# LucaHermes/ddrl

Hardware: AMD Instinct MI355X
Metric: env-steps/sec at 4096 envs × 4 leg agents; PPO update ms/minibatch (higher is better)
Workload: dtype fp32

## Files before the change

### ddrl_amd/csrc/ppo_ffn_impl.h

```cpp
#pragma once
#include <atomic>
#include "common.h"
#include "kernels.h"
#include "ffn.h"
#include "ppo_loss.h"

#ifndef DDRL_FFN_AT
#define DDRL_FFN_AT 0
#endif

#ifndef DDRL_FFN_KSP
#define DDRL_FFN_KSP 0
#endif
#if DDRL_FFN_KSP == 1
#define DDRL_FFN_LAUNCH launch_update_ffn_k1
#elif DDRL_FFN_AT == 2
#define DDRL_FFN_LAUNCH launch_update_ffn_peer
#elif DDRL_FFN_AT
#define DDRL_FFN_LAUNCH launch_update_ffn_atomic
#else
#define DDRL_FFN_LAUNCH launch_update_ffn
#endif
#if DDRL_FFN_AT || defined(DDRL_XCHG_ATOMIC)
#define DDRL_XCHG_IS_ATOMIC 1
#else
#define DDRL_XCHG_IS_ATOMIC 0
#endif
#define DDRL_XCHG_LXSYS (DDRL_FFN_AT == 2)
#define DDRL_LX_ON (!DDRL_XCHG_IS_ATOMIC || DDRL_XCHG_LXSYS)

namespace {

typedef float float2v __attribute__((ext_vector_type(2)));

template <int NW, int ROWS>
struct Geo {
  static constexpr int NT = 64 * NW;
  static constexpr int RT = ROWS / (16 * NW);
  static constexpr int NS1 = 16 / NW;
  static constexpr int NS2 = (12 + NW - 1) / NW;
};
__host__ __device__ constexpr int waves_for(int A, int ksp) { return ksp == 2 ? 4 : (A == 8 ? 4 : 8); }
__host__ __device__ constexpr int ncup_slots(int OB, bool pol) { return pol && OB == 4 ? 2 * OB : 0; }
__host__ __device__ constexpr int gx_pairs(int OB, int NW) {
  return ((64 * OB + OB + 128 + ncup_slots(OB, true) + 64 * NW - 1) / (64 * NW) + 2) / 2 + 2 * (16 / NW + (12 + NW - 1) / NW);
}
#define GX_MAX_PAIRS 20

struct UpdateBatch {
  UpdateArgs a[DDRL_MAXP];
  UpdateHyper h;
  int nrows;
  float inv_n;
  unsigned long long* xchg;
  unsigned long long* gx;
  int* err;
  int* xcc;
  unsigned epoch;
  unsigned lds_bytes;
  int own_kq;
  unsigned lx_base;
};

#ifdef DDRL_BOUNDS
__device__ unsigned g_bounds[DDRL_NBOUNDS];
__device__ __forceinline__ bool bchk(bool ok, int k) {
  if (!ok) atomicAdd(&g_bounds[k], 1u);
  return ok;
}
}
#if !DDRL_FFN_AT
#if DDRL_FFN_KSP == 2
extern "C" int ddrl_diag_bounds_k1(unsigned* host, int reset);
#endif
#if DDRL_FFN_KSP == 1
extern "C" int ddrl_diag_bounds_k1(unsigned* host, int reset) {
#else
extern "C" int ddrl_diag_bounds(unsigned* host, int reset) {
#endif
  if (hipMemcpyFromSymbol(host, HIP_SYMBOL(g_bounds), sizeof(g_bounds)) != hipSuccess) return -1;
  if (reset) {
    unsigned z[DDRL_NBOUNDS] = {0};
    if (hipMemcpyToSymbol(HIP_SYMBOL(g_bounds), z, sizeof(z)) != hipSuccess) return -1;
  }
#if DDRL_FFN_KSP == 2
  unsigned k1[DDRL_NBOUNDS];
  if (ddrl_diag_bounds_k1(k1, reset) != 0) return -1;
  for (int i = 0; i < DDRL_NBOUNDS; ++i) host[i] += k1[i];
#endif
  return 0;
}
#endif
namespace {
#define BCHK(cond, k) bchk((cond), (k))
#else
#define BCHK(cond, k) true
#endif
__device__ __forceinline__ unsigned xchg_tag(unsigned epoch, int step) {
  return (epoch << 20) | (((unsigned)step + 1u) & 0xfffffu);
}

struct BranchOff { int w1, b1, w2, b2, wo, bo, cup; };
__device__ __forceinline__ BranchOff branch_off(const FfnOffsets& o, bool pol) {
  BranchOff b;
  b.cup = o.n;
  b.w1 = pol ? o.w1 : o.vw1; b.b1 = pol ? o.b1 : o.vb1;
  b.w2 = pol ? o.w2 : o.vw2; b.b2 = pol ? o.b2 : o.vb2;
  b.wo = pol ? o.wo : o.vo;  b.bo = pol ? o.bo : o.vbo;
  return b;
}

template <int OB, bool PAD>
__device__ void stage_branch(const float* __restrict__ th, int d, const BranchOff& bo, float* lds,
                             NetLds& W, int ncup) {
  W.w1 = lds; W.w2 = W.w1 + lds_img(48, PAD); W.b1 = W.w2 + lds_img(64, PAD); W.b2 = W.b1 + 64;
  W.wo = W.b2 + 64; W.bo = W.wo + 64 * OB; W.cup = W.bo + OB;
  for (int i = threadIdx.x; i < ncup; i += blockDim.x) W.cup[i] = th[bo.cup + i];
  for (int i = threadIdx.x; i < 48 * 64; i += blockDim.x) {
    const int f = i >> 6;
    W.w1[sidx<PAD>(f, i & 63)] = f < d ? th[bo.w1 + i] : 0.f;
  }
  for (int i = threadIdx.x; i < 64 * 64; i += blockDim.x) W.w2[sidx<PAD>(i >> 6, i & 63)] = th[bo.w2 + i];
  for (int i = threadIdx.x; i < 64; i += blockDim.x) { W.b1[i] = th[bo.b1 + i]; W.b2[i] = th[bo.b2 + i]; }
  for (int i = threadIdx.x; i < 64 * OB; i += blockDim.x) W.wo[i] = th[bo.wo + i];
  for (int i = threadIdx.x; i < OB; i += blockDim.x) W.bo[i] = th[bo.bo + i];
}
template <int OB, int NT, bool PAD>
__device__ __forceinline__ void stage_branch_batched(const float* __restrict__ th, int d, const BranchOff& bo,
                                                     float* lds, NetLds& W, int ncup) {
  static_assert((48 * 64) % NT == 0 && (64 * 64) % NT == 0, "staging split");
  constexpr int N1 = 48 * 64 / NT, N2 = 64 * 64 / NT, NS = (64 * OB + OB + 128 + NT - 1) / NT;
  W.w1 = lds; W.w2 = W.w1 + lds_img(48, PAD); W.b1 = W.w2 + lds_img(64, PAD); W.b2 = W.b1 + 64;
  W.wo = W.b2 + 64; W.bo = W.wo + 64 * OB; W.cup = W.bo + OB;
  const int t = threadIdx.x;
  float a1[N1], a2[N2], as[NS];
#pragma unroll
  for (int k = 0; k < N1; ++k) {
    const int i = t + NT * k;
    a1[k] = (i >> 6) < d ? th[bo.w1 + i] : 0.f;
  }
#pragma unroll
  for (int k = 0; k < N2; ++k) a2[k] = th[bo.w2 + t + NT * k];
#pragma unroll
  for (int k = 0; k < NS; ++k) {
    int e = t + NT * k;
    float x = 0.f;
    if (e < 64 * OB) x = th[bo.wo + e];
    else if ((e -= 64 * OB) < OB) x = th[bo.bo + e];
    else if ((e -= OB) < 64) x = th[bo.b1 + e];
    else if ((e -= 64) < 64) x = th[bo.b2 + e];
    as[k] = x;
  }
  float ac = t < ncup ? th[bo.cup + t] : 0.f;
#pragma unroll
  for (int k = 0; k < N1; ++k) {
    const int i = t + NT * k;
    W.w1[sidx<PAD>(i >> 6, i & 63)] = a1[k];
  }
#pragma unroll
  for (int k = 0; k < N2; ++k) {
    const int i = t + NT * k;
    W.w2[sidx<PAD>(i >> 6, i & 63)] = a2[k];
  }
#pragma unroll
  for (int k = 0; k < NS; ++k) {
    int e = t + NT * k;
    if (e < 64 * OB) W.wo[e] = as[k];
    else if ((e -= 64 * OB) < OB) W.bo[e] = as[k];
    else if ((e -= OB) < 64) W.b1[e] = as[k];
    else if ((e -= 64) < 64) W.b2[e] = as[k];
  }
  if (t < ncup) W.cup[t] = ac;
}
__host__ __device__ constexpr int branch_lds_floats(bool pad) { return lds_img(48, pad) + lds_img(64, pad) + 128 + 64 * 16 + 16; }
__host__ __device__ constexpr bool update_pad(int A, int ksp) { return kLdsPad && !(A == 8 && ksp == 1); }

template <int OB>
__device__ __forceinline__ void small_param(int e, const BranchOff& bo, const NetLds& W, int& pidx, float*& lp) {
  if (e < 64 * OB) { pidx = bo.wo + e; lp = W.wo + e; return; }
  e -= 64 * OB;
  if (e < OB) { pidx = bo.bo + e; lp = W.bo + e; return; }
  e -= OB;
  if (e < 64) { pidx = bo.b1 + e; lp = W.b1 + e; return; }
  e -= 64;
  if (e < 64) { pidx = bo.b2 + e; lp = W.b2 + e; return; }
  e -= 64;
  pidx = bo.cup + e; lp = W.cup + e;
}


template <int A, int RT>
struct RowData {
  float x[RT][12];
  float act[RT][A];
  float ol[RT][2 * A];
  float s0[RT], s1[RT];
  int cid[RT];
};

template <int NW, int ROWS>
__device__ __forceinline__ void issue_rows(const float* rec, int stride, int cpr, int cpr_l, float inv_cpr_l,
                                           const int* idxb, float* stg, int R, unsigned lds_bytes) {
  const int lane = threadIdx.x & 63, w = __builtin_amdgcn_readfirstlane(threadIdx.x >> 6);
  if (w == NW - 1) return;
  constexpr int MI = (ROWS * 20 + 64 * (NW - 1) - 1) / (64 * (NW - 1));
  const int nchunk = ROWS * cpr_l;
  int idx[MI], kk[MI];
#pragma unroll
  for (int it = 0; it < MI; ++it) {
    const int g = 64 * w + 64 * (NW - 1) * it + lane;
    int row = (int)(((float)g + 0.5f) * inv_cpr_l);
    kk[it] = min(g - row * cpr_l, cpr - 1);
    idx[it] = 0;
    if (g < nchunk) {
      if (!BCHK(row >= 0 && row < ROWS && kk[it] >= 0, 0)) row = 0;
      idx[it] = idxb[row];
    }
  }
#pragma unroll
  for (int it = 0; it < MI; ++it) {
    const int base = 64 * w + 64 * (NW - 1) * it;
    if (base >= nchunk) break;
    const unsigned dst = __builtin_amdgcn_readfirstlane(lds_addr(stg + 4 * base));
    if (base + lane < nchunk) {
      int i = idx[it];
      if (!BCHK(i >= 0 && i < R, 1)) i = 0;
      if (BCHK(dst + 16u * (unsigned)lane + 16u <= lds_bytes, 3))
        glds16(rec + (size_t)i * stride + 4 * kk[it], dst);
    }
  }
  (void)R; (void)lds_bytes;
}

__host__ __device__ constexpr int stg_chunks(int stride, int A) { return A == 8 ? stride / 4 : (stride / 4) | 1; }

template <int A, int KS1, bool POL, int RT>
__device__ __forceinline__ void load_row(const float* stg, int stg_stride, const RecLayout& L, const int* row_l,
                                         int d, RowData<A, RT>& r, unsigned xlast_bits = 0xffffffffu) {
  const int q = (threadIdx.x & 63) >> 4;
#ifdef DDRL_BOUNDS
  {
    int hi = KS1 < 12 ? L.obs + 4 * KS1 - 1 : L.obs + d - 1;
    if (POL) hi = max(max(hi, L.act + A - 1), max(L.logit + 2 * A - 1, max(L.logp, max(L.adv, L.cid))));
    else hi = max(hi, max(L.vf, L.vt));
    for (int t = 0; t < RT; ++t) BCHK(row_l[t] >= 0 && row_l[t] < DDRL_MB && hi < L.stride, 4);
  }
#endif
#pragma unroll
  for (int t = 0; t < RT; ++t) {
    const float* rp = stg + row_l[t] * stg_stride;
#pragma unroll
    for (int s = 0; s < 12; ++s)
      r.x[t][s] = (s < KS1 && (KS1 < 12 || 4 * s + q < d)) ? rp[L.obs + 4 * s + q] : 0.f;
    if (KS1 < 12) r.x[t][KS1 - 1] = __uint_as_float(__float_as_uint(r.x[t][KS1 - 1]) & xlast_bits);
    if (POL) {
#pragma unroll
      for (int j = 0; j < A; ++j) r.act[t][j] = rp[L.act + j];
#pragma unroll
      for (int j = 0; j < 2 * A; ++j) r.ol[t][j] = rp[L.logit + j];
      r.s0[t] = rp[L.logp];
      r.s1[t] = rp[L.adv];
      r.cid[t] = L.cid >= 0 ? min(max((int)rp[L.cid], 0), 3) : 0;
    } else {
      r.cid[t] = 0;
#pragma unroll
      for (int j = 0; j < A; ++j) r.act[t][j] = 0.f;
#pragma unroll
      for (int j = 0; j < 2 * A; ++j) r.ol[t][j] = 0.f;
      r.s0[t] = rp[L.vf];
      r.s1[t] = rp[L.vt];
    }
  }
}

template <bool POL, int NSTAT, int NW, int KSP>
__device__ __forceinline__ void write_stats(float* so, const float* red, float inv_n) {
  float sv[NSTAT];
#pragma unroll
  for (int k = 0; k < NSTAT; ++k) {
    if constexpr (KSP == 2) {
      sv[k] = red[96 + k];
    } else {
      sv[k] = 0.f;
      for (int i = 0; i < NW; ++i) sv[k] += red[i * 8 + k];
    }
  }
  if constexpr (POL) {
    gst(so + 1, sv[0] * inv_n); gst(so + 3, sv[1] * inv_n); gst(so + 4, sv[2] * inv_n);
  } else {
    gst(so + 2, sv[0] * inv_n);
    const float vy = sv[2] * inv_n - (sv[1] * inv_n) * (sv[1] * inv_n);
    const float vd = sv[4] * inv_n - (sv[3] * inv_n) * (sv[3] * inv_n);
    gst(so + 5, vy > 0.f ? fmaxf(-1.f, 1.f - vd / vy) : 0.f);
  }
}

__device__ __forceinline__ int row_index(const UpdateArgs& U, int step, int row_l, bool ok) {
  if (!ok) return 0;
  if (!U.shuffle) return row_l;
  const int e = step / U.nb, b = step - e * U.nb;
#ifdef DDRL_BOUNDS
  if (!BCHK(e >= 0 && e < U.n_epochs, 2)) return 0;
  const int slot = gld(U.perm + e * U.nb + b);
  if (!BCHK(slot >= 0 && slot < U.nb && (slot + 1) * DDRL_MB <= max(U.R, DDRL_MB) && row_l < DDRL_MB, 2)) return 0;
  return gld(U.shuffle + slot * DDRL_MB + row_l);
#else
  return gld(U.shuffle + gld(U.perm + e * U.nb + b) * DDRL_MB + row_l);
#endif
}
__device__ __forceinline__ int perm_slot(const UpdateArgs& U, int step) {
  const int e = step / U.nb, b = step - e * U.nb;
  return gld(U.perm + e * U.nb + b);
}

#ifdef DDRL_STAMPS
__device__ unsigned long long g_stamps[32][16];
#define STAMP_INIT unsigned long long st_prev = __builtin_amdgcn_s_memtime(), st_acc[16] = {0};
#ifndef DDRL_STAMP_TID
#define DDRL_STAMP_TID 0
#endif
#define STAMP(k) do { if (tid == DDRL_STAMP_TID) { const unsigned long long t_ = __builtin_amdgcn_s_memtime(); st_acc[k] += t_ - st_prev; st_prev = t_; } } while (0)
#define STAMP_DONE do { if (tid == DDRL_STAMP_TID) for (int k_ = 0; k_ < 16; ++k_) g_stamps[blockIdx.x][k_] = st_acc[k_]; } while (0)
}
#if !DDRL_FFN_AT && DDRL_FFN_KSP != 1
extern "C" int ddrl_diag_stamps(unsigned long long* host) {
  return hipMemcpyFromSymbol(host, HIP_SYMBOL(g_stamps), sizeof(g_stamps)) == hipSuccess ? 0 : -1;
}
#endif
namespace {
#else
#define STAMP_INIT
#define STAMP(k)
#define STAMP_DONE
#endif

constexpr int kGxSt = 0, kGxLd = 16;
#define XCHG_SLOW_TICKS 20000ull
#define XCHG_TIMEOUT_TICKS 300000000ull
__device__ __forceinline__ bool xchg_abandon(unsigned long long t0, int* err) {
  const unsigned long long dt = __builtin_amdgcn_s_memrealtime() - t0;
  if (dt < XCHG_SLOW_TICKS) return false;
  if (__hip_atomic_load(err, __ATOMIC_RELAXED, __HIP_MEMORY_SCOPE_AGENT)) return true;
  if (dt > XCHG_TIMEOUT_TICKS) { atomicExch(err, 1); return true; }
  return false;
}
#if DDRL_XCHG_IS_ATOMIC
#define DDRL_XCHG_SCOPE __HIP_MEMORY_SCOPE_SYSTEM
typedef unsigned long long* gx_box_t;
__device__ __forceinline__ gx_box_t gx_rsrc(unsigned long long* box) { return box; }
__device__ __forceinline__ void gx_put(gx_box_t r, int j, float v0, float v1, unsigned tag, bool) {
  unsigned long long* g = r + 2 * (j * 256 + (int)threadIdx.x);
  __hip_atomic_store(g, ((unsigned long long)tag << 32) | __float_as_uint(v0), __ATOMIC_RELAXED, DDRL_XCHG_SCOPE);
  __hip_atomic_store(g + 1, ((unsigned long long)tag << 32) | __float_as_uint(v1), __ATOMIC_RELAXED,
                     DDRL_XCHG_SCOPE);
}
__device__ __forceinline__ void xchg_store(unsigned long long* g, unsigned long long v, bool) {
  __hip_atomic_store(g, v, __ATOMIC_RELAXED, DDRL_XCHG_SCOPE);
}
__device__ __forceinline__ unsigned long long xchg_load(unsigned long long* g) {
  return __hip_atomic_load(g, __ATOMIC_RELAXED, DDRL_XCHG_SCOPE);
}
template <int NP, typename F>
__device__ __forceinline__ bool gx_get(gx_box_t r, unsigned tag, float* out, int* err, F&& after_first) {
  bool lost = false;
  unsigned long long g[2 * NP];
  unsigned long long* b = r + 2 * (int)threadIdx.x;
  const unsigned long long t0 = __builtin_amdgcn_s_memrealtime();
  bool first = true;
  for (;;) {
#pragma unroll
    for (int j = 0; j < NP; ++j) {
      g[2 * j] = __hip_atomic_load(b + 512 * j, __ATOMIC_RELAXED, DDRL_XCHG_SCOPE);
      g[2 * j + 1] = __hip_atomic_load(b + 512 * j + 1, __ATOMIC_RELAXED, DDRL_XCHG_SCOPE);
    }
    if (first) { after_first(); first = false; }
    bool ok = true;
#pragma unroll
    for (int j = 0; j < 2 * NP; ++j) ok = ok && (unsigned)(g[j] >> 32) == tag;
    if (ok) break;
    if (xchg_abandon(t0, err)) {
#pragma unroll
      for (int j = 0; j < 2 * NP; ++j) g[j] = 0ull;
      lost = true;
      break;
    }
    __builtin_amdgcn_s_sleep(1);
  }
#pragma unroll
  for (int j = 0; j < 2 * NP; ++j) out[j] = __uint_as_float((unsigned)g[j]);
  return lost;
}
#else
typedef __amdgpu_buffer_rsrc_t gx_box_t;
__device__ __forceinline__ gx_box_t gx_rsrc(unsigned long long* box) {
  return __builtin_amdgcn_make_buffer_rsrc(box, 0, GX_MAX_PAIRS * 256 * 16, 0x00020000);
}
__device__ __forceinline__ void gx_put(gx_box_t r, int j, float v0, float v1, unsigned tag, bool coh) {
  const v4u g = {__float_as_uint(v0), tag, __float_as_uint(v1), tag};
  if (coh) __builtin_amdgcn_raw_buffer_store_b128(g, r, (j * 256 + (int)threadIdx.x) * 16, 0, 16);
  else __builtin_amdgcn_raw_buffer_store_b128(g, r, (j * 256 + (int)threadIdx.x) * 16, 0, kGxSt);
}
__device__ __forceinline__ void xchg_store(unsigned long long* g, unsigned long long v, bool coh) {
  const __amdgpu_buffer_rsrc_t r = __builtin_amdgcn_make_buffer_rsrc(g, 0, 8, 0x00020000);
  typedef unsigned v2u_t __attribute__((ext_vector_type(2)));
  const v2u_t x = {(unsigned)v, (unsigned)(v >> 32)};
  if (coh) __builtin_amdgcn_raw_buffer_store_b64(x, r, 0, 0, 16);
  else __builtin_amdgcn_raw_buffer_store_b64(x, r, 0, 0, kGxSt);
}
__device__ __forceinline__ unsigned long long xchg_load(unsigned long long* g) {
  const __amdgpu_buffer_rsrc_t r = __builtin_amdgcn_make_buffer_rsrc(g, 0, 8, 0x00020000);
  typedef unsigned v2u_t __attribute__((ext_vector_type(2)));
  const v2u_t x = __builtin_amdgcn_raw_buffer_load_b64(r, 0, 0, kGxLd);
  return ((unsigned long long)x[1] << 32) | x[0];
}
template <int NP, typename F>
__device__ __forceinline__ bool gx_get(gx_box_t r, unsigned tag, float* out, int* err, F&& after_first) {
  bool lost = false;
  v4u g[NP];
  const unsigned long long t0 = __builtin_amdgcn_s_memrealtime();
  bool first = true;
  for (;;) {
#pragma unroll
    for (int j = 0; j < NP; ++j) g[j] = __builtin_amdgcn_raw_buffer_load_b128(r, (j * 256 + (int)threadIdx.x) * 16, 0, kGxLd);
    if (first) { after_first(); first = false; }
    bool ok = true;
#pragma unroll
    for (int j = 0; j < NP; ++j) ok = ok && g[j][1] == tag && g[j][3] == tag;
    if (ok) break;
    if (xchg_abandon(t0, err)) {
#pragma unroll
      for (int j = 0; j < NP; ++j) g[j] = v4u{0u, 0u, 0u, 0u};
      lost = true;
      break;
    }
    __builtin_amdgcn_s_sleep(1);
  }
#pragma unroll
  for (int j = 0; j < NP; ++j) {
    out[2 * j] = __uint_as_float(g[j][0]);
    out[2 * j + 1] = __uint_as_float(g[j][2]);
  }
  return lost;
}
#endif

__device__ __forceinline__ unsigned lx_bit(int step) { return ((unsigned)(step >> 1) & 1u) ^ 1u; }
__device__ __forceinline__ float lx_t(float v, unsigned bit) { return __uint_as_float((__float_as_uint(v) & ~1u) | bit); }
#if DDRL_LX_ON
#if DDRL_XCHG_LXSYS
typedef __amdgpu_buffer_rsrc_t lx_box_t;
__device__ __forceinline__ lx_box_t lx_rsrc(unsigned long long* box) {
  return __builtin_amdgcn_make_buffer_rsrc(box, 0, GX_MAX_PAIRS * 256 * 16, 0x00020000);
}
constexpr int kLxSt = 17, kLxLd = 17;
#else
typedef gx_box_t lx_box_t;
__device__ __forceinline__ lx_box_t lx_rsrc(unsigned long long* box) { return gx_rsrc(box); }
constexpr int kLxSt = kGxSt, kLxLd = kGxLd;
#endif
__device__ __forceinline__ void gx_put4(lx_box_t r, int j, float a, float b, float c, float d, unsigned bit) {
  const v4u g = {__float_as_uint(lx_t(a, bit)), __float_as_uint(lx_t(b, bit)), __float_as_uint(lx_t(c, bit)),
                 __float_as_uint(lx_t(d, bit))};
  __builtin_amdgcn_raw_buffer_store_b128(g, r, (j * 256 + (int)threadIdx.x) * 16, 0, kLxSt);
}
template <int NQ, typename F>
__device__ __forceinline__ bool gx_get4(lx_box_t r, unsigned bit, float* out, int* err, F&& after_first) {
  bool lost = false;
  v4u g[NQ];
  const unsigned long long t0 = __builtin_amdgcn_s_memrealtime();
  bool first = true;
  for (;;) {
#pragma unroll
    for (int j = 0; j < NQ; ++j) g[j] = __builtin_amdgcn_raw_buffer_load_b128(r, (j * 256 + (int)threadIdx.x) * 16, 0, kLxLd);
    if (first) { after_first(); first = false; }
    unsigned bad = 0;
#pragma unroll
    for (int j = 0; j < NQ; ++j) bad |= (g[j][0] ^ bit) | (g[j][1] ^ bit) | (g[j][2] ^ bit) | (g[j][3] ^ bit);
    if ((bad & 1u) == 0) break;
    if (xchg_abandon(t0, err)) {
#pragma unroll
      for (int j = 0; j < NQ; ++j) g[j] = v4u{0u, 0u, 0u, 0u};
      lost = true;
      break;
    }
    __builtin_amdgcn_s_sleep(1);
  }
#pragma unroll
  for (int j = 0; j < NQ; ++j)
#pragma unroll
    for (int k = 0; k < 4; ++k) out[4 * j + k] = __uint_as_float(g[j][k]);
  return lost;
}
#endif

template <int O>
__device__ __forceinline__ void head_bwd_mfma(const NetLds& W, const float* dout, floatx4 dh[4]) {
  static_assert(O % 4 == 0, "policy head: 2A outputs");
  const int lane = threadIdx.x & 63, c = lane & 15, q = lane >> 4;
  float b[O / 4];
#pragma unroll
  for (int kk = 0; kk < O / 4; ++kk)
    b[kk] = q == 0 ? dout[4 * kk] : q == 1 ? dout[4 * kk + 1] : q == 2 ? dout[4 * kk + 2] : dout[4 * kk + 3];
#pragma unroll
  for (int fb = 0; fb < 4; ++fb) {
    floatx4 acc = splat4(0.f);
#pragma unroll
    for (int kk = 0; kk < O / 4; ++kk) acc = mfma4(W.wo[(16 * fb + c) * O + 4 * kk + q], b[kk], acc);
    dh[fb] = acc;
  }
}

template <int NROWS, int NT_, int LD = NROWS + 8>
__device__ __forceinline__ void dw_tiles_fm_head(const float* A, const float* B, const int* fa, int fo, floatx4* out,
                                                 const float* AH, const float* BH, int fah, floatx4& outh) {
  const int lane = threadIdx.x & 63, c = lane & 15, q = lane >> 4;
#pragma unroll
  for (int i = 0; i < NT_; ++i) out[i] = splat4(0.f);
  outh = splat4(0.f);
  const float* bp = B + (16 * fo + c) * LD + 4 * q;
  const float* bph = BH + c * LD + 4 * q;
  const float* aph = AH + (16 * fah + c) * LD + 4 * q;
  const float* ap[NT_];
#pragma unroll
  for (int i = 0; i < NT_; ++i) ap[i] = A + (16 * fa[i] + c) * LD + 4 * q;
  constexpr int NU = NROWS / 16;
  floatx4 bv[2], av[2][NT_], bhv[2], ahv[2];
  bv[0] = *reinterpret_cast<const floatx4*>(bp);
  bhv[0] = *reinterpret_cast<const floatx4*>(bph);
  ahv[0] = *reinterpret_cast<const floatx4*>(aph);
#pragma unroll
  for (int i = 0; i < NT_; ++i) av[0][i] = *reinterpret_cast<const floatx4*>(ap[i]);
#pragma unroll
  for (int u = 0; u < NU; ++u) {
    if (u + 1 < NU) {
      bv[(u + 1) & 1] = *reinterpret_cast<const floatx4*>(bp + 16 * (u + 1));
      bhv[(u + 1) & 1] = *reinterpret_cast<const floatx4*>(bph + 16 * (u + 1));
      ahv[(u + 1) & 1] = *reinterpret_cast<const floatx4*>(aph + 16 * (u + 1));
#pragma unroll
      for (int i = 0; i < NT_; ++i) av[(u + 1) & 1][i] = *reinterpret_cast<const floatx4*>(ap[i] + 16 * (u + 1));
    }
#pragma unroll
    for (int v = 0; v < 4; ++v) {
#pragma unroll
      for (int i = 0; i < NT_; ++i) out[i] = mfma4(av[u & 1][i][v], bv[u & 1][v], out[i]);
      outh = mfma4(ahv[u & 1][v], bhv[u & 1][v], outh);
    }
    __builtin_amdgcn_sched_barrier(0);
  }
}

template <int A, int KS1, int OB, bool POL, int NW, int KSP, bool CUP, bool LSBX>
__device__ __forceinline__ void update_loop(const UpdateArgs& U, const UpdateBatch& ub, float* lds, int p, int kq) {
  constexpr int ROWS = DDRL_MB / KSP;
  constexpr int NT = Geo<NW, ROWS>::NT, RT = Geo<NW, ROWS>::RT, NS1 = Geo<NW, ROWS>::NS1, NS2 = Geo<NW, ROWS>::NS2;
  constexpr bool PAD = update_pad(A, KSP);
  const int wkq = ub.own_kq < 0 ? 0 : ub.own_kq;
  const UpdateHyper& H = ub.h;
  const int d = U.d;
  const FfnOffsets of = ffn_offsets(d, A);
  const BranchOff bo = branch_off(of, POL);
  const int nf1 = (d + 15) >> 4;
  constexpr int NSB0 = 64 * OB + OB + 128;
  constexpr int NCUP = CUP ? ncup_slots(OB, POL) : 0;
  constexpr int NSB = NSB0 + NCUP;
  constexpr bool cup = NCUP > 0;
  constexpr int nsb = NSB;
  constexpr int NSLOT = (NSB + NT - 1) / NT;
  constexpr int NSTAT = POL ? 3 : 5;
  constexpr int NTS = NS1 + NS2;
  constexpr int NP0 = (NSLOT + 2) / 2;
  constexpr int NP = NP0 + 2 * NTS;
  static_assert(KSP == 1 || (NT == 256 && NP == gx_pairs(OB, NW) && NP <= GX_MAX_PAIRS), "exchange pairs");
  constexpr bool LX = LSBX && KSP == 2 && DDRL_LX_ON;
  constexpr int NQ0 = (NSLOT + 1 + 3) / 4;
  constexpr int NQ = NQ0 + NTS;
  static_assert(!LX || NQ <= GX_MAX_PAIRS, "exchange quads");

  NetLds W;
  constexpr int LD = ROWS + 8;
  float* bufA = lds + branch_lds_floats(PAD);
  float* bufB = bufA + 64 * LD;
  float* Pb = bufB + 64 * LD;
  float* red = Pb + NW * NSB;
  int* idxb = reinterpret_cast<int*>(red + 128);
  constexpr bool HMF = POL && KSP == 2;
  float* bufH = red + 256;
  float* bufD = bufH + 64 * LD;
  float* stg = red + 256 + (HMF ? 80 * LD : 0);
  const int stride = U.lay.stride, cpr = stride >> 2, cpr_l = stg_chunks(stride, A);
  const float inv_cpr_l = 1.f / (float)cpr_l;

  const int tid = threadIdx.x, lane = tid & 63, c = lane & 15, q = lane >> 4,
            w = __builtin_amdgcn_readfirstlane(tid >> 6);
  constexpr bool coh = false;
  int row_l[RT];
  bool row_ok[RT];
#pragma unroll
  for (int t = 0; t < RT; ++t) {
    row_l[t] = 16 * RT * w + 16 * t + c;
    row_ok[t] = ROWS * kq + row_l[t] < ub.nrows;
  }

  const int total_steps = U.n_epochs * U.nb;
  const int last = U.max_steps >= 0 ? min(total_steps, U.step0 + U.max_steps) : total_steps;
  const int gr = ROWS * kq + tid;
  const bool gok = tid < ROWS && gr < ub.nrows;
  if (tid < ROWS) idxb[tid] = U.step0 < last && gok ? row_index(U, U.step0, gr, true) : 0;
  __syncthreads();
  if (U.step0 < last) issue_rows<NW, ROWS>(U.rec, stride, cpr, cpr_l, inv_cpr_l, idxb, stg, U.R, ub.lds_bytes);
  stage_branch_batched<OB, NT, PAD>(U.theta, d, bo, lds, W, NCUP);
  if constexpr (HMF) {
    for (int i = tid; i < NW * NSB; i += NT) Pb[i] = 0.f;
    for (int i = tid; i < 16 * LD; i += NT) bufD[i] = 0.f;
  }

  floatx4 mt[NTS], vt4[NTS];
  bool tv[NTS];
  int tfa[NTS], tfo[NTS];
#pragma unroll
  for (int i = 0; i < NTS; ++i) {
    const int tt = i < NS1 ? w + NW * i : w + NW * (i - NS1);
    tv[i] = i < NS1 ? true : (tt < 4 * nf1);
    tfa[i] = tt >> 2;
    tfo[i] = tt & 3;
#pragma unroll
    for (int r = 0; r < 4; ++r) {
      const int f = 16 * tfa[i] + 4 * q + r, o = 16 * tfo[i] + c;
      const bool ok = tv[i] && (i < NS1 || f < d) && !U.grad_out;
      const int pidx = (i < NS1 ? bo.w2 : bo.w1) + f * 64 + o;
      BCHK(!ok || (pidx >= 0 && pidx < of.n), 5);
      mt[i][r] = ok ? U.m[pidx] : 0.f;
      vt4[i][r] = ok ? U.v[pidx] : 0.f;

    }
  }
  float ms[NSLOT], vs[NSLOT];
  int sp_pidx[NSLOT], sp_lds[NSLOT];
#pragma unroll
  for (int k = 0; k < NSLOT; ++k) {
    const int e = tid + NT * k;
    ms[k] = vs[k] = 0.f;
    sp_pidx[k] = 0;
    sp_lds[k] = (int)(red + 127 - lds);
    if (e < nsb) {
      int pidx; float* lp;
      small_param<OB>(e, bo, W, pidx, lp);
      BCHK(pidx >= 0 && pidx < of.n + NCUP, 5);
      sp_pidx[k] = pidx;
      sp_lds[k] = (int)(lp - lds);
      if (!U.grad_out) {
        ms[k] = U.m[pidx];
        vs[k] = U.v[pidx];
      }
    }
  }
  int ebase[4];
#pragma unroll
  for (int r = 0; r < 4; ++r) ebase[r] = sidx<PAD>(4 * q + r, 16 * (w & 3) + c);
  float b1p = U.beta_pow[0], b2p = U.beta_pow[1];
  const float adv_mean = U.adv_norm[0], adv_den = U.adv_norm[1];
  const float beta = U.kl_coeff;
  const float lo = 1.f - H.clip, hi = 1.f + H.clip;
  __syncthreads();

  RowData<A, RT> cur;
  const unsigned xlast_bits = (KS1 < 12 && 4 * (KS1 - 1) + q >= d) ? 0u : 0xffffffffu;
  wait_vmcnt0();
  __syncthreads();
  if (tid < ROWS) idxb[tid] = U.step0 + 1 < last && gok ? row_index(U, U.step0 + 1, gr, true) : 0;
  int nxt = U.step0 + 2 < last && gok ? row_index(U, U.step0 + 2, gr, true) : 0;
  const size_t gx_branch = ((size_t)p * 2 + (POL ? 0 : 1)) * KSP;
  __syncthreads();

  const float inv_rows = 1.f / (float)ub.nrows;
  STAMP_INIT
  for (int step = U.step0; step < last; ++step) {
    const float alpha = H.lr * sqrtf(1.f - b2p) / (1.f - b1p);
    load_row<A, KS1, POL, RT>(stg, 4 * cpr_l, U.lay, row_l, d, cur, xlast_bits);
    floatx4 h1[RT][4], h2[RT][4], dz[RT][4];
    float out[RT][OB], dout[RT][OB];
    ffn_fwd_rt<OB, KS1, RT, PAD>(W, cur.x, h1, h2, out);
    float pre[RT][A], cf[RT][A];
    if constexpr (cup) {
      {
#pragma unroll
        for (int t = 0; t < RT; ++t)
#pragma unroll
          for (int j = 0; j < A; ++j) {
            pre[t][j] = out[t][j];
            cf[t][j] = W.cup[cur.cid[t] * A + j];
            out[t][j] *= cf[t][j];
          }
      }
    }
    STAMP(0);
    float st[NSTAT];
#pragma unroll
    for (int k = 0; k < NSTAT; ++k) st[k] = 0.f;
#pragma unroll
    for (int t = 0; t < RT; ++t) {
      float st0[NSTAT];
      if constexpr (POL)
        policy_loss_row<A>(out[t], cur.act[t], cur.ol[t], cur.s0[t], (cur.s1[t] - adv_mean) / adv_den,
                           beta, lo, hi, H.ent_coeff, ub.inv_n, row_ok[t], dout[t], st0);
      else
        value_loss_row(out[t][0], cur.s0[t], cur.s1[t], H, ub.inv_n, row_ok[t], dout[t], st0);
#pragma unroll
      for (int k = 0; k < NSTAT; ++k) st[k] += st0[k];
    }
    STAMP(1);
    float* Pw = Pb + w * NSB;
    if constexpr (cup) {
      {
#pragma unroll
        for (int lg = 0; lg < 4; ++lg)
#pragma unroll
          for (int j = 0; j < A; ++j) {
            float v = 0.f;
#pragma unroll
            for (int t = 0; t < RT; ++t) v += cur.cid[t] == lg ? dout[t][j] * pre[t][j] : 0.f;
            v = row16_sum(v);
            if (lane == 0) Pw[NSB0 + lg * A + j] = v;
          }
#pragma unroll
        for (int t = 0; t < RT; ++t)
#pragma unroll
          for (int j = 0; j < A; ++j) dout[t][j] *= cf[t][j];
      }
    }
    const int h_own = 16 * (c >> 2) + 4 * q + (c & 3);
    if constexpr (HMF) {
#pragma unroll
      for (int t = 0; t < RT; ++t) {
        store_act_fm<LD>(bufH, RT * w + t, h2[t]);
        if (q == 0)
#pragma unroll
          for (int o = 0; o < OB; ++o) bufD[o * LD + row_l[t]] = dout[t][o];
      }
    }
#ifndef DDRL_ABL_NO_HEADDPP
#pragma unroll
    for (int o = 0; o < (HMF ? 0 : OB); ++o) {
      float v[16];
#pragma unroll
      for (int fb = 0; fb < 4; ++fb)
#pragma unroll
        for (int r = 0; r < 4; ++r) {
          v[4 * fb + r] = h2[0][fb][r] * dout[0][o];
#pragma unroll
          for (int t = 1; t < RT; ++t) v[4 * fb + r] += h2[t][fb][r] * dout[t][o];
        }
      Pw[h_own * OB + o] = row16_transpose_sum(v);
    }
#endif
#pragma unroll
    for (int o = 0; o < OB; ++o) {
      float dsum = dout[0][o];
#pragma unroll
      for (int t = 1; t < RT; ++t) dsum += dout[t][o];
      const float s = row16_sum(dsum);
      if (lane == 0) Pw[64 * OB + o] = s;
    }
#pragma unroll
    for (int k = 0; k < NSTAT; ++k) {
      const float s = row16_sum(st[k]);
      if (lane == 0) red[w * 8 + k] = s;
    }
    STAMP(2);
#pragma unroll
    for (int t = 0; t < RT; ++t) {
      if constexpr (POL) head_bwd_mfma<OB>(W, dout[t], dz[t]);
      else head_bwd<OB>(W, dout[t], dz[t]);
      dtanh_inplace(dz[t], h2[t]);
    }
    {
      float v[16];
#pragma unroll
      for (int fb = 0; fb < 4; ++fb)
#pragma unroll
        for (int r = 0; r < 4; ++r) {
          v[4 * fb + r] = dz[0][fb][r];
#pragma unroll
          for (int t = 1; t < RT; ++t) v[4 * fb + r] += dz[t][fb][r];
        }
      Pw[64 * OB + OB + 64 + h_own] = row16_transpose_sum(v);
    }
#pragma unroll
    for (int t = 0; t < RT; ++t) {
      store_act_fm<LD>(bufA, RT * w + t, h1[t]);
      store_act_fm<LD>(bufB, RT * w + t, dz[t]);
    }
    STAMP(3);
#ifndef DDRL_ABL_NO_L2BWD
    layer2_bwd_rt<RT, PAD>(W, dz, h2);
#endif
#pragma unroll
    for (int t = 0; t < RT; ++t) dtanh_inplace(h2[t], h1[t]);
    {
      float v[16];
#pragma unroll
      for (int fb = 0; fb < 4; ++fb)
#pragma unroll
        for (int r = 0; r < 4; ++r) {
          v[4 * fb + r] = h2[0][fb][r];
#pragma unroll
          for (int t = 1; t < RT; ++t) v[4 * fb + r] += h2[t][fb][r];
        }
      Pw[64 * OB + OB + h_own] = row16_transpose_sum(v);
    }
    STAMP(4);
    __syncthreads();
    STAMP(5);
    const unsigned gtag = xchg_tag(ub.epoch, step);
    const int gstep = step + (int)ub.lx_base;
    const unsigned lbit = lx_bit(gstep);
    (void)lbit;
    const size_t gx_box = (size_t)GX_MAX_PAIRS * 256 * 2;
    const gx_box_t gx_mine = gx_rsrc(ub.gx + ((gx_branch + kq) * 2 + (gstep & 1)) * gx_box);
    float gs[NSLOT];
    float st_own = 0.f;
    auto put_small = [&] {
      float v0[2 * NP0];
#pragma unroll
      for (int k = 0; k < 2 * NP0; ++k) v0[k] = 0.f;
#pragma unroll
      for (int k = 0; k < NSLOT; ++k) {
        const int e = tid + NT * k;
        float sm = 0.f;
        if (e < nsb)
          for (int i = 0; i < NW; ++i) sm += Pb[i * NSB + e];
        gs[k] = sm;
        v0[k] = sm;
      }
      if (tid < NSTAT)
        for (int i = 0; i < NW; ++i) st_own += red[i * 8 + tid];
      v0[NSLOT] = st_own;
#if DDRL_LX_ON
      if constexpr (LX) {
        const lx_box_t lx_mine = lx_rsrc(ub.gx + ((gx_branch + kq) * 2 + (gstep & 1)) * gx_box);
        float w0[4 * NQ0];
#pragma unroll
        for (int k = 0; k < 4 * NQ0; ++k) w0[k] = k <= NSLOT ? v0[k] : 0.f;
#pragma unroll
        for (int j = 0; j < NQ0; ++j) gx_put4(lx_mine, j, w0[4 * j], w0[4 * j + 1], w0[4 * j + 2], w0[4 * j + 3], lbit);
        return;
      }
#endif
#pragma unroll
      for (int j = 0; j < NP0; ++j) gx_put(gx_mine, j, v0[2 * j], v0[2 * j + 1], gtag, coh);
    };
    if constexpr (KSP == 2 && !HMF) put_small();
    floatx4 gt[NTS];
#ifndef DDRL_ABL_NO_DW2
    if constexpr (HMF) {
      static_assert(NW == 4, "one head tile (16 features) per wave");
      floatx4 gh;
      dw_tiles_fm_head<ROWS, NS1, ROWS + 8>(bufA, bufB, tfa, w & 3, gt, bufH, bufD, w, gh);
      if (c < OB)
#pragma unroll
        for (int r = 0; r < 4; ++r) Pb[(16 * w + 4 * q + r) * OB + c] = gh[r];
    } else {
      dw_tiles_fm<ROWS, NS1, ROWS + 8>(bufA, bufB, tfa, w & 3, gt);
    }
#else
    for (int i = 0; i < NS1; ++i) gt[i] = splat4(0.f);
#endif
    if constexpr (KSP == 2) {
#pragma unroll
      for (int i = 0; i < NS1; ++i) {
#if DDRL_LX_ON
        if constexpr (LX) {
          gx_put4(lx_rsrc(ub.gx + ((gx_branch + kq) * 2 + (gstep & 1)) * gx_box), NQ0 + i, gt[i][0], gt[i][1], gt[i][2],
                  gt[i][3], lbit);
          continue;
        }
#endif
        gx_put(gx_mine, NP0 + 2 * i, gt[i][0], gt[i][1], gtag, coh);
        gx_put(gx_mine, NP0 + 2 * i + 1, gt[i][2], gt[i][3], gtag, coh);
      }
    }
    STAMP(6);
    __syncthreads();
    if constexpr (HMF) put_small();
    STAMP(7);
#pragma unroll
    for (int t = 0; t < RT; ++t) {
      store_act_fm<LD>(bufB, RT * w + t, h2[t]);
#pragma unroll
      for (int s = 0; s < 12; ++s) bufA[(4 * s + q) * LD + row_l[t]] = cur.x[t][s];
    }
    __syncthreads();
    STAMP(8);
#ifndef DDRL_ABL_NO_PREFETCH
    if (KSP == 1 && step + 1 < last) issue_rows<NW, ROWS>(U.rec, stride, cpr, cpr_l, inv_cpr_l, idxb, stg, U.R, ub.lds_bytes);
#endif
    const int xlane = 64 * (NW - 1);
    unsigned long long* const xmine = ub.xchg + (((size_t)p * 2 + (POL ? 0 : 1)) * KSP + kq) * 2 + (step & 1);
    unsigned long long* const xother = ub.xchg + (((size_t)p * 2 + (POL ? 1 : 0)) * KSP + kq) * 2 + (step & 1);
    unsigned long long xv = 0;
    if (tid == xlane) xv = xchg_load(xother);
    STAMP(9);
    {
#pragma unroll
      for (int i = NS1; i < NTS; ++i) gt[i] = splat4(0.f);
      int n1 = 0;
#pragma unroll
      for (int i = NS1; i < NTS; ++i) n1 += tv[i] ? 1 : 0;
#ifdef DDRL_ABL_NO_DW1
      n1 = -1;
#endif
      if (n1 == NS2) dw_tiles_fm<ROWS, NS2, ROWS + 8>(bufA, bufB, tfa + NS1, w & 3, gt + NS1);
      else if constexpr (NS2 >= 3) {
        if (n1 == 2) dw_tiles_fm<ROWS, 2, ROWS + 8>(bufA, bufB, tfa + NS1, w & 3, gt + NS1);
        else if (n1 == 1) dw_tiles_fm<ROWS, 1, ROWS + 8>(bufA, bufB, tfa + NS1, w & 3, gt + NS1);
      } else if (n1 == 1) dw_tiles_fm<ROWS, 1, ROWS + 8>(bufA, bufB, tfa + NS1, w & 3, gt + NS1);
    }
    STAMP(10);
    if constexpr (KSP == 2) {
#pragma unroll
      for (int i = NS1; i < NTS; ++i) {
#if DDRL_LX_ON
        if constexpr (LX) {
          gx_put4(lx_rsrc(ub.gx + ((gx_branch + kq) * 2 + (gstep & 1)) * gx_box), NQ0 + i, gt[i][0], gt[i][1], gt[i][2],
                  gt[i][3], lbit);
          continue;
        }
#endif
        gx_put(gx_mine, NP0 + 2 * i, gt[i][0], gt[i][1], gtag, coh);
        gx_put(gx_mine, NP0 + 2 * i + 1, gt[i][2], gt[i][3], gtag, coh);
      }
#if DDRL_LX_ON
      if constexpr (LX) {
        float o4[4 * NQ];
        gx_get4<NQ>(lx_rsrc(ub.gx + ((gx_branch + (kq ^ 1)) * 2 + (gstep & 1)) * gx_box), lbit, o4, ub.err, [&] {
          if (step + 1 < last) issue_rows<NW, ROWS>(U.rec, stride, cpr, cpr_l, inv_cpr_l, idxb, stg, U.R, ub.lds_bytes);
        });
#pragma unroll
        for (int k = 0; k < NSLOT; ++k) gs[k] = lx_t(gs[k], lbit) + o4[k];
        if (tid < NSTAT) red[96 + tid] = lx_t(st_own, lbit) + o4[NSLOT];
#pragma unroll
        for (int i = 0; i < NTS; ++i)
#pragma unroll
          for (int r = 0; r < 4; ++r) gt[i][r] = lx_t(gt[i][r], lbit) + o4[4 * (NQ0 + i) + r];
      } else
#endif
      {
      float o[2 * NP];
#ifndef DDRL_ABL_NO_PREFETCH
      gx_get<NP>(gx_rsrc(ub.gx + ((gx_branch + (kq ^ 1)) * 2 + (gstep & 1)) * gx_box), gtag, o, ub.err, [&] {
        if (step + 1 < last) issue_rows<NW, ROWS>(U.rec, stride, cpr, cpr_l, inv_cpr_l, idxb, stg, U.R, ub.lds_bytes);
      });
#else
      gx_get<NP>(gx_rsrc(ub.gx + ((gx_branch + (kq ^ 1)) * 2 + (gstep & 1)) * gx_box), gtag, o, ub.err, [] {});
#endif
      if constexpr (LSBX) {
#pragma unroll
        for (int k = 0; k < NSLOT; ++k) gs[k] = lx_t(gs[k], lbit) + lx_t(o[k], lbit);
        if (tid < NSTAT) red[96 + tid] = lx_t(st_own, lbit) + lx_t(o[NSLOT], lbit);
#pragma unroll
        for (int i = 0; i < NTS; ++i)
#pragma unroll
          for (int r = 0; r < 4; ++r) gt[i][r] = lx_t(gt[i][r], lbit) + lx_t(o[2 * NP0 + 4 * i + r], lbit);
      } else {
#pragma unroll
        for (int k = 0; k < NSLOT; ++k) gs[k] += o[k];
        if (tid < NSTAT) red[96 + tid] = st_own + o[NSLOT];
#pragma unroll
        for (int i = 0; i < NTS; ++i)
#pragma unroll
          for (int r = 0; r < 4; ++r) gt[i][r] += o[2 * NP0 + 4 * i + r];
      }
      }
      STAMP(14);
    } else {
#pragma unroll
      for (int k = 0; k < NSLOT; ++k) {
        const int e = tid + NT * k;
        float sm = 0.f;
        if (e < nsb)
          for (int i = 0; i < NW; ++i) sm += Pb[i * NSB + e];
        gs[k] = sm;
      }
    }
    float ss = 0.f;
#pragma unroll
    for (int k = 0; k < NSLOT; ++k) ss += gs[k] * gs[k];
#pragma unroll
    for (int i = 0; i < NTS; ++i)
#pragma unroll
      for (int r = 0; r < 4; ++r) {
        if (tv[i]) ss += gt[i][r] * gt[i][r];
      }

    if (U.grad_out) {
#pragma unroll
      for (int i = 0; i < NTS; ++i)
#pragma unroll
        for (int r = 0; r < 4; ++r) {
          const int f = 16 * tfa[i] + 4 * q + r, o = 16 * tfo[i] + c;
          if (tv[i] && (i < NS1 || f < d)) U.grad_out[(i < NS1 ? bo.w2 : bo.w1) + f * 64 + o] = gt[i][r];
        }
#pragma unroll
      for (int k = 0; k < NSLOT; ++k) {
        const int e = tid + NT * k;
        if (e < nsb) U.grad_out[sp_pidx[k]] = gs[k];
      }
      if (U.stats) {
        __syncthreads();
        if (tid == 64) write_stats<POL, NSTAT, NW, KSP>(U.stats + (size_t)step * 8, red, inv_rows);
      }
      return;
    }

    ss = wave_sum(ss);
    if (lane == 0) red[64 + w] = ss;
    __syncthreads();
    if (tid == xlane) {
      float local = 0.f;
      for (int i = 0; i < NW; ++i) local += red[64 + i];
      const unsigned tag = xchg_tag(ub.epoch, step);
      xchg_store(xmine, ((unsigned long long)tag << 32) | __float_as_uint(local), coh);
      unsigned long long v = xv;
      const unsigned long long t0 = __builtin_amdgcn_s_memrealtime();
#ifdef DDRL_ABL_NO_EXCHANGE
      v = ((unsigned long long)tag << 32) | __float_as_uint(local);
#endif
      while ((unsigned)(v >> 32) != tag) {
        v = xchg_load(xother);
        if ((unsigned)(v >> 32) == tag) break;
        if (xchg_abandon(t0, ub.err)) break;
        __builtin_amdgcn_s_sleep(1);
      }
      const float partner = __uint_as_float((unsigned)(v & 0xffffffffu));
      const float tot = local + partner;
      const float gn = __builtin_amdgcn_sqrtf(tot);
      red[80] = gn;
      red[81] = H.grad_clip * fminf(__builtin_amdgcn_rcpf(gn), 1.f / H.grad_clip);
    }
    __syncthreads();
    STAMP(11);
    auto stats_out = [&] {
      write_stats<POL, NSTAT, NW, KSP>(U.stats + (size_t)step * 8, red, inv_rows);
      gst(U.stats + (size_t)step * 8 + 6, red[80]);
      gst(U.stats + (size_t)step * 8 + 7, red[81]);
    };
    if (KSP == 1 && U.stats && tid == 64 && kq == wkq) stats_out();
    const float scale = red[81];
    const float c1 = 1.f - H.b1, c2 = 1.f - H.b2;

#ifndef DDRL_ABL_NO_ADAM
    {
      float th[NTS][4], ts[NSLOT];
#pragma unroll
      for (int i = 0; i < NTS; ++i)
#pragma unroll
        for (int r = 0; r < 4; ++r)
          th[i][r] = (i < NS1 ? W.w2 : W.w1)[ebase[r] + lds_blk(PAD) * tfa[i]];
#pragma unroll
      for (int k = 0; k < NSLOT; ++k) ts[k] = lds[sp_lds[k]];
#pragma unroll
      for (int i = 0; i < NTS; ++i)
#pragma unroll
        for (int h = 0; h < 2; ++h) {
          const float2v gr = {gt[i][2 * h], gt[i][2 * h + 1]};
          float2v m2 = {mt[i][2 * h], mt[i][2 * h + 1]}, v2 = {vt4[i][2 * h], vt4[i][2 * h + 1]};
          const float2v sc = {scale, scale}, k1 = {c1, c1}, k2 = {c2, c2}, al = {alpha, alpha};
          const float2v g = gr * sc;
          m2 = __builtin_elementwise_fma(__builtin_elementwise_fma(gr, sc, -m2), k1, m2);
          v2 = __builtin_elementwise_fma(__builtin_elementwise_fma(g, g, -v2), k2, v2);
          float2v den = {__builtin_amdgcn_sqrtf(v2[0]), __builtin_amdgcn_sqrtf(v2[1])};
          den = den + (float2v){H.eps, H.eps};
          const float2v rc = {__builtin_amdgcn_rcpf(den[0]), __builtin_amdgcn_rcpf(den[1])};
          const float2v t2 = __builtin_elementwise_fma(-(m2 * al), rc, (float2v){th[i][2 * h], th[i][2 * h + 1]});
          mt[i][2 * h] = m2[0]; mt[i][2 * h + 1] = m2[1];
          vt4[i][2 * h] = v2[0]; vt4[i][2 * h + 1] = v2[1];
          th[i][2 * h] = t2[0]; th[i][2 * h + 1] = t2[1];
        }

#pragma unroll
      for (int k = 0; k < NSLOT; ++k) {
        const float g = gs[k] * scale;
        ms[k] = ms[k] + (g - ms[k]) * c1;
        vs[k] = vs[k] + (g * g - vs[k]) * c2;
        ts[k] = ts[k] - (ms[k] * alpha) * __builtin_amdgcn_rcpf(__builtin_amdgcn_sqrtf(vs[k]) + H.eps);
      }
#pragma unroll
      for (int i = 0; i < NTS; ++i)
#pragma unroll
        for (int r = 0; r < 4; ++r) {
          if (tv[i]) (i < NS1 ? W.w2 : W.w1)[ebase[r] + lds_blk(PAD) * tfa[i]] = th[i][r];
        }
#pragma unroll
      for (int k = 0; k < NSLOT; ++k) lds[sp_lds[k]] = ts[k];
    }
#endif
    b1p = b1p * H.b1;
    b2p = b2p * H.b2;
    STAMP(12);
    wait_vmcnt0();
    if (tid < ROWS) idxb[tid] = nxt;
    __syncthreads();
    if (tid < ROWS) nxt = step + 3 < last && gok ? row_index(U, step + 3, gr, true) : 0;
    if (KSP == 2 && U.stats && tid == 64 && kq == wkq) stats_out();
    STAMP(13);
  }
  STAMP_DONE;
  if (U.grad_out || kq != wkq) return;
  if (__hip_atomic_load(ub.err, __ATOMIC_RELAXED, __HIP_MEMORY_SCOPE_AGENT)) return;

#pragma unroll
  for (int i = 0; i < NTS; ++i)
#pragma unroll
    for (int r = 0; r < 4; ++r) {
      const int f = 16 * tfa[i] + 4 * q + r, o = 16 * tfo[i] + c;
      if (!(tv[i] && (i < NS1 || f < d))) continue;
      const int pidx = (i < NS1 ? bo.w2 : bo.w1) + f * 64 + o;
      U.m[pidx] = mt[i][r];
      U.v[pidx] = vt4[i][r];
    }
#pragma unroll
  for (int k = 0; k < NSLOT; ++k) {
    const int e = tid + NT * k;
    if (e >= nsb) continue;
    int pidx; float* lp;
    small_param<OB>(e, bo, W, pidx, lp);
    U.m[pidx] = ms[k];
    U.v[pidx] = vs[k];
    U.theta[pidx] = *lp;
  }
  for (int i = tid; i < 48 * 64; i += NT) {
    const int f = i >> 6;
    if (f < d) U.theta[bo.w1 + i] = W.w1[sidx<PAD>(f, i & 63)];
  }
  for (int i = tid; i < 64 * 64; i += NT) U.theta[bo.w2 + i] = W.w2[sidx<PAD>(i >> 6, i & 63)];
  if (POL && tid == 0) {
    U.beta_pow[0] = b1p;
    U.beta_pow[1] = b2p;
  }
}

template <int A, int KS1, int KSP, bool CUP, bool LSBX>
__global__ void __launch_bounds__(64 * waves_for(A, KSP)) k_update_ffn(UpdateBatch ub) {
  extern __shared__ float lds[];
  constexpr int NW = waves_for(A, KSP);
  const int p = blockIdx.x & 7;
  if (threadIdx.x == 0) {
    unsigned x;
    asm volatile("s_getreg_b32 %0, hwreg(HW_REG_XCC_ID)" : "=s"(x));
    ub.xcc[blockIdx.x] = (int)(x & 0xf);
  }
  if (p >= ub.h.P) return;
  const int j = blockIdx.x >> 3, branch = j / KSP, kq = j - branch * KSP;
  if (ub.own_kq >= 0 && kq != ub.own_kq) return;
  const UpdateArgs U = ub.a[p];
  if (branch) update_loop<A, KS1, 1, false, NW, KSP, false, LSBX>(U, ub, lds, p, kq);
  else update_loop<A, KS1, 2 * A, true, NW, KSP, CUP, LSBX>(U, ub, lds, p, kq);
}

static size_t update_lds_bytes(int O, int stride, int ksp) {
  const int nsb = 64 * O + O + 128 + ncup_slots(O, true);
  const int nw = waves_for(O / 2, ksp);
  return (size_t)(branch_lds_floats(update_pad(O / 2, ksp)) + 2 * 64 * (DDRL_MB / ksp + 8) + nw * nsb + 256 +
                  (ksp == 2 ? 80 * (DDRL_MB / ksp + 8) : 0) +
                  (DDRL_MB / ksp) * 4 * stg_chunks(stride, O / 2)) * 4;
}

template <int A, int KS1, bool CUP = false>
static void launch_update_t(hipStream_t s, UpdateBatch& ub, int P, int stride, int ksp, bool lx) {
  ub.lds_bytes = (unsigned)update_lds_bytes(2 * A, stride, ksp);
#if DDRL_FFN_KSP != 1
  if (ksp == 2 && lx)
    hipLaunchKernelGGL((k_update_ffn<A, KS1, 2, CUP, true>), dim3(24 + P), dim3(64 * waves_for(A, 2)), ub.lds_bytes, s, ub);
#endif
#if DDRL_FFN_KSP != 2
  if (ksp == 2 && !lx)
    hipLaunchKernelGGL((k_update_ffn<A, KS1, 2, CUP, false>), dim3(24 + P), dim3(64 * waves_for(A, 2)), ub.lds_bytes, s, ub);
  if (ksp == 1)
    hipLaunchKernelGGL((k_update_ffn<A, KS1, 1, CUP, false>), dim3(8 + P), dim3(64 * waves_for(A, 1)), ub.lds_bytes, s, ub);
#endif
}

}

void DDRL_FFN_LAUNCH(hipStream_t s, const UpdateArgs* ua, const UpdateHyper& h, int nrows, float inv_n,
                       int A, int d, int stride, int cup, unsigned long long* xchg, unsigned long long* gx, int ksp,
                       int* err, unsigned* epoch_ctr, int* xcc, int own_kq, unsigned lx_base) {
#if DDRL_FFN_KSP == 2
  if (!(ksp == 2 && ua[0].grad_out == nullptr)) {
    launch_update_ffn_k1(s, ua, h, nrows, inv_n, A, d, stride, cup, xchg, gx, ksp, err, epoch_ctr, xcc, own_kq, lx_base);
    return;
  }
#endif
  UpdateBatch ub;
  for (int p = 0; p < DDRL_MAXP; ++p) ub.a[p] = p < h.P ? ua[p] : UpdateArgs{};
  ub.h = h;
  ub.nrows = nrows;
  ub.inv_n = inv_n;
  ub.xchg = xchg;
  ub.gx = gx;
  ub.err = err;
  ub.xcc = xcc;
  ub.own_kq = own_kq;
  ub.lx_base = lx_base;
  ub.epoch = (*epoch_ctr)++ % 4095u + 1u;
  const bool lx = ksp == 2 && ua[0].grad_out == nullptr;
  if (ub.epoch == 1) (void)hipMemsetAsync(xchg, 0, sizeof(unsigned long long) * 8 * DDRL_MAXP, s);
  if (own_kq < 0 && (ub.epoch == 1 || (lx && DDRL_LX_ON))) {
    const int s0 = ua[0].step0;
    const unsigned b0 = (((unsigned)s0 >> 1) & 1u) ^ 1u, b1 = (((unsigned)(s0 + 1) >> 1) & 1u) ^ 1u;
    if (!(lx && DDRL_LX_ON) || (b0 && b1)) {
      (void)hipMemsetAsync(gx, 0, gx_bytes(DDRL_MAXP), s);
    } else {
      const size_t box = sizeof(unsigned long long) * (size_t)GX_MAX_PAIRS * 256 * 2;
      const size_t nbox = gx_bytes(DDRL_MAXP) / box;
      for (int q = 0; q < 2; ++q) {
        const unsigned first_bit = (s0 & 1) == q ? b0 : b1;
        (void)hipMemset2DAsync(reinterpret_cast<char*>(gx) + q * box, 2 * box, first_bit ? 0 : 1, box, nbox / 2, s);
      }
    }
  }
  if (cup)
    launch_update_t<2, 5, true>(s, ub, h.P, stride, ksp, lx);
  else
    DDRL_DISPATCH_A_KS1(A, d, launch_update_t, s, ub, h.P, stride, ksp, lx);
}
```

Baseline: 1.208 million.

## Split row prefetch into address prep during exchange poll and later fire

```diff
diff --git a/ddrl_amd/csrc/ppo_ffn_impl.h b/ddrl_amd/csrc/ppo_ffn_impl.h
--- a/ddrl_amd/csrc/ppo_ffn_impl.h
+++ b/ddrl_amd/csrc/ppo_ffn_impl.h
@@ -199,11 +199,18 @@
 };
 
 template <int NW, int ROWS>
-__device__ __forceinline__ void issue_rows(const float* rec, int stride, int cpr, int cpr_l, float inv_cpr_l,
-                                           const int* idxb, float* stg, int R, unsigned lds_bytes) {
+struct RowGather {
+  static constexpr int MI = (ROWS * 20 + 64 * (NW - 1) - 1) / (64 * (NW - 1));
+  const float* src[MI];
+};
+template <int NW, int ROWS>
+__device__ __forceinline__ void rows_prepare(RowGather<NW, ROWS>& G, const float* rec, int stride, int cpr, int cpr_l,
+                                             float inv_cpr_l, const int* idxb, int R) {
+  constexpr int MI = RowGather<NW, ROWS>::MI;
   const int lane = threadIdx.x & 63, w = __builtin_amdgcn_readfirstlane(threadIdx.x >> 6);
+#pragma unroll
+  for (int it = 0; it < MI; ++it) G.src[it] = rec;
   if (w == NW - 1) return;
-  constexpr int MI = (ROWS * 20 + 64 * (NW - 1) - 1) / (64 * (NW - 1));
   const int nchunk = ROWS * cpr_l;
   int idx[MI], kk[MI];
 #pragma unroll
@@ -219,17 +226,36 @@
   }
 #pragma unroll
   for (int it = 0; it < MI; ++it) {
+    int i = idx[it];
+    if (64 * w + 64 * (NW - 1) * it + lane < nchunk && !BCHK(i >= 0 && i < R, 1)) i = 0;
+    G.src[it] = rec + (size_t)i * stride + 4 * kk[it];
+  }
+  (void)R;
+}
+template <int NW, int ROWS>
+__device__ __forceinline__ void rows_fire(const RowGather<NW, ROWS>& G, int cpr_l, float* stg, unsigned lds_bytes) {
+  constexpr int MI = RowGather<NW, ROWS>::MI;
+  const int lane = threadIdx.x & 63, w = __builtin_amdgcn_readfirstlane(threadIdx.x >> 6);
+  if (w == NW - 1) return;
+  const int nchunk = ROWS * cpr_l;
+  const unsigned stg_a = lds_addr(stg);
+#pragma unroll
+  for (int it = 0; it < MI; ++it) {
     const int base = 64 * w + 64 * (NW - 1) * it;
     if (base >= nchunk) break;
-    const unsigned dst = __builtin_amdgcn_readfirstlane(lds_addr(stg + 4 * base));
+    const unsigned dst = __builtin_amdgcn_readfirstlane(stg_a + 16u * (unsigned)base);
     if (base + lane < nchunk) {
-      int i = idx[it];
-      if (!BCHK(i >= 0 && i < R, 1)) i = 0;
-      if (BCHK(dst + 16u * (unsigned)lane + 16u <= lds_bytes, 3))
-        glds16(rec + (size_t)i * stride + 4 * kk[it], dst);
-    }
-  }
-  (void)R; (void)lds_bytes;
+      if (BCHK(dst + 16u * (unsigned)lane + 16u <= lds_bytes, 3)) glds16(G.src[it], dst);
+    }
+  }
+  (void)lds_bytes;
+}
+template <int NW, int ROWS>
+__device__ __forceinline__ void issue_rows(const float* rec, int stride, int cpr, int cpr_l, float inv_cpr_l,
+                                           const int* idxb, float* stg, int R, unsigned lds_bytes) {
+  RowGather<NW, ROWS> G;
+  rows_prepare<NW, ROWS>(G, rec, stride, cpr, cpr_l, inv_cpr_l, idxb, R);
+  rows_fire<NW, ROWS>(G, cpr_l, stg, lds_bytes);
 }
 
 __host__ __device__ constexpr int stg_chunks(int stride, int A) { return A == 8 ? stride / 4 : (stride / 4) | 1; }
@@ -315,16 +341,21 @@
 
 #ifdef DDRL_STAMPS
 __device__ unsigned long long g_stamps[32][16];
+__device__ unsigned g_poll_stale[32][8];
 #define STAMP_INIT unsigned long long st_prev = __builtin_amdgcn_s_memtime(), st_acc[16] = {0};
 #ifndef DDRL_STAMP_TID
 #define DDRL_STAMP_TID 0
 #endif
 #define STAMP(k) do { if (tid == DDRL_STAMP_TID) { const unsigned long long t_ = __builtin_amdgcn_s_memtime(); st_acc[k] += t_ - st_prev; st_prev = t_; } } while (0)
-#define STAMP_DONE do { if (tid == DDRL_STAMP_TID) for (int k_ = 0; k_ < 16; ++k_) g_stamps[blockIdx.x][k_] = st_acc[k_]; } while (0)
+#define STAMP_DONE do { if (tid == DDRL_STAMP_TID) for (int k_ = 0; k_ < 16; ++k_) g_stamps[blockIdx.x][k_] = st_acc[k_]; \
+                        if (lane == 0) g_poll_stale[blockIdx.x][w & 7] = st_stale; } while (0)
 }
 #if !DDRL_FFN_AT && DDRL_FFN_KSP != 1
 extern "C" int ddrl_diag_stamps(unsigned long long* host) {
   return hipMemcpyFromSymbol(host, HIP_SYMBOL(g_stamps), sizeof(g_stamps)) == hipSuccess ? 0 : -1;
+}
+extern "C" int ddrl_diag_poll_stale(unsigned* host) {
+  return hipMemcpyFromSymbol(host, HIP_SYMBOL(g_poll_stale), sizeof(g_poll_stale)) == hipSuccess ? 0 : -1;
 }
 #endif
 namespace {
@@ -491,6 +522,54 @@
     for (int k = 0; k < 4; ++k) out[4 * j + k] = __uint_as_float(g[j][k]);
   return lost;
 }
+#if !DDRL_XCHG_LXSYS
+#define DDRL_LX_ASMPOLL 1
+template <int NQ, typename F>
+__device__ __forceinline__ bool gx_get4c(unsigned long long* box, unsigned bit, float* out, int* err, unsigned& stale,
+                                         F&& after_first) {
+  bool lost = false;
+  v4u g[NQ];
+  const unsigned long long ba = (unsigned long long)box;
+  const v4u rs = {(unsigned)__builtin_amdgcn_readfirstlane((int)(unsigned)ba),
+                  (unsigned)__builtin_amdgcn_readfirstlane((int)((unsigned)(ba >> 32) & 0xffffu)),
+                  (unsigned)(GX_MAX_PAIRS * 256 * 16), 0x00020000u};
+  const unsigned voff = (unsigned)threadIdx.x * 16u;
+  const unsigned long long t0 = __builtin_amdgcn_s_memrealtime();
+  bool first = true;
+  for (;;) {
+#pragma unroll
+    for (int j = 0; j < NQ; ++j)
+      asm volatile("buffer_load_dwordx4 %0, %1, %2, %3 offen sc1" : "=v"(g[j]) : "v"(voff), "s"(rs), "s"(j * 4096));
+    __builtin_amdgcn_sched_barrier(0);
+    if (first) after_first();
+    __builtin_amdgcn_sched_barrier(0);
+    asm volatile("s_waitcnt vmcnt(0)" ::: "memory");
+#pragma unroll
+    for (int j = 0; j < NQ; ++j) asm volatile("" : "+v"(g[j]));
+    unsigned bad = 0;
+#pragma unroll
+    for (int j = 0; j < NQ; ++j) bad |= (g[j][0] ^ bit) | (g[j][1] ^ bit) | (g[j][2] ^ bit) | (g[j][3] ^ bit);
+#ifdef DDRL_STAMPS
+    if (first && __builtin_amdgcn_ballot_w64((bad & 1u) != 0)) ++stale;
+#endif
+    first = false;
+    if ((bad & 1u) == 0) break;
+    if (xchg_abandon(t0, err)) {
+#pragma unroll
+      for (int j = 0; j < NQ; ++j) g[j] = v4u{0u, 0u, 0u, 0u};
+      lost = true;
+      break;
+    }
+    __builtin_amdgcn_s_sleep(1);
+  }
+  (void)stale;
+#pragma unroll
+  for (int j = 0; j < NQ; ++j)
+#pragma unroll
+    for (int k = 0; k < 4; ++k) out[4 * j + k] = __uint_as_float(g[j][k]);
+  return lost;
+}
+#endif
 #endif
 
 template <int O>
@@ -673,6 +752,8 @@
   __syncthreads();
 
   const float inv_rows = 1.f / (float)ub.nrows;
+  unsigned st_stale = 0;
+  (void)st_stale;
   STAMP_INIT
   for (int step = U.step0; step < last; ++step) {
     const float alpha = H.lr * sqrtf(1.f - b2p) / (1.f - b1p);
@@ -851,6 +932,8 @@
     };
     if constexpr (KSP == 2 && !HMF) put_small();
     floatx4 gt[NTS];
+    RowGather<NW, ROWS> G;
+    (void)G;
 #ifndef DDRL_ABL_NO_DW2
     if constexpr (HMF) {
       static_assert(NW == 4, "one head tile (16 features) per wave");
@@ -932,9 +1015,16 @@
 #if DDRL_LX_ON
       if constexpr (LX) {
         float o4[4 * NQ];
+#ifdef DDRL_LX_ASMPOLL
+        asm volatile("" : "+v"(xv));
+        gx_get4c<NQ>(ub.gx + ((gx_branch + (kq ^ 1)) * 2 + (gstep & 1)) * gx_box, lbit, o4, ub.err, st_stale, [&] {
+          rows_prepare<NW, ROWS>(G, U.rec, stride, cpr, cpr_l, inv_cpr_l, idxb, U.R);
+        });
+#else
         gx_get4<NQ>(lx_rsrc(ub.gx + ((gx_branch + (kq ^ 1)) * 2 + (gstep & 1)) * gx_box), lbit, o4, ub.err, [&] {
           if (step + 1 < last) issue_rows<NW, ROWS>(U.rec, stride, cpr, cpr_l, inv_cpr_l, idxb, stg, U.R, ub.lds_bytes);
         });
+#endif
 #pragma unroll
         for (int k = 0; k < NSLOT; ++k) gs[k] = lx_t(gs[k], lbit) + o4[k];
         if (tid < NSTAT) red[96 + tid] = lx_t(st_own, lbit) + o4[NSLOT];
@@ -1015,6 +1105,10 @@
     ss = wave_sum(ss);
     if (lane == 0) red[64 + w] = ss;
     __syncthreads();
+#ifdef DDRL_LX_ASMPOLL
+    if constexpr (LX)
+      if (step + 1 < last) rows_fire<NW, ROWS>(G, cpr_l, stg, ub.lds_bytes);
+#endif
     if (tid == xlane) {
       float local = 0.f;
       for (int i = 0; i < NW; ++i) local += red[64 + i];
```

After: 1.244 million, median of 6. 1.03x the previous value.
